# REXJJ/high-fidelity-pointcloud-fusion

Measured on AMD Instinct MI355X. Metric: Mpts/s fused into 1 mm voxel grid, higher is better.
Workload: dtype f64

## Files before the change

### high-fidelity-pointcloud-fusion_amd/csrc/hfpf.hip

```cpp
#include <hip/hip_runtime.h>

#include <cstring>

#include <rocprim/rocprim.hpp>

#include <dlfcn.h>
#include <sched.h>
#include <sys/mman.h>

#if !defined(__HIP_DEVICE_COMPILE__)
#include <emmintrin.h>
#endif
#include <algorithm>
#include <atomic>
#include <condition_variable>
#include <cmath>
#include <cstdarg>
#include <cstdio>
#include <cstdlib>
#include <cstring>
#include <mutex>
#include <string>
#include <thread>
#include <vector>
// ... 115 lines not shown
                }
            }
            if (stop_.load(std::memory_order_acquire)) return;
            seen = g;
            part(i);
            remaining_.fetch_sub(1, std::memory_order_acq_rel);
        }
    }
    std::vector<std::thread> th_;
    std::mutex m_;
    std::condition_variable cv_;
    std::atomic<uint64_t> gen_{0};
    std::atomic<int> remaining_{0}, sleepers_{0};
    std::atomic<bool> stop_{false};
    char* dst_ = nullptr;
    const char* src_ = nullptr;
    size_t bytes_ = 0;
};

constexpr int kStageSlots = 8;
constexpr size_t kXferChunk = 16u << 20;
#ifndef HFPF_PROBE_FRAMES
#define HFPF_PROBE_FRAMES 8
#endif
constexpr int kProbeFrames = HFPF_PROBE_FRAMES;
constexpr int kFrameSlots = 8;

struct DepthSpec {
    uint32_t width, height, depth_f32, depth_step, color_bpp, color_bgr, color_step;
    float cx, cy, sx, sy, unit;
    uint32_t color_off;
    size_t depth_bytes() const { return (size_t)(height - 1) * depth_step + (size_t)width * (depth_f32 ? 4u : 2u); }
    size_t color_bytes() const { return color_bpp ? (size_t)(height - 1) * color_step + (size_t)width * color_bpp : 0; }
};
static_assert(sizeof(DepthSpec) == 13 * 4, "DepthSpec is compared bytewise");

DepthLayout depth_layout(const DepthSpec& d, const void* dev_color, uint64_t color_stride)
{
    return DepthLayout{d.color_bpp ? (const uint8_t*)dev_color : nullptr, color_stride, d.width, d.depth_step, d.color_step, d.depth_f32,
                       d.color_bpp, d.color_bgr, d.cx, d.cy, d.sx, d.sy, d.unit};
}

struct Knobs {
    int copy_streams = 2;
    bool update_cells = true;
    int host_batch = 4;
    int upd_shape_forced = -1;
    bool trace_shape = false;
    bool bin_spare = true;
    bool stream_replay = true;
    float bin_slack = 2.0f;
    bool clean_small_nowait = true;
    bool clean_overlap = true;
    bool trace_clean = false;
    float test_bin_scale = 1.f;
    bool test_table_skip = false;
    bool mailbox = true;
    int test_dev_tile = kDevTileDefault;
    int stage_threads = 0;
};

struct Session {
    bool dirty = false;
    uint64_t n_linked[kLogRegions] = {0};
    uint64_t gate_done = 0;
    bool pend_valid = false;
    uint64_t direct_linked = 0;
    bool normals_possible = false;
    uint32_t next_frame_id = 0;
    bool poisoned = false;
    std::string poison_msg;
    bool bin_have_hist = false;
    bool bin_from_probe = false;
    double bin_prev_points = 0;
    uint64_t n_bricks_known = 0;
    uint64_t n_bricks_before = 0;
    unsigned long long upd_miss_seen = 0, upd_member_seen = 0;
    unsigned long long pub_seq = 0;
    unsigned long long early_seq = 0;
    unsigned long long win_seq = 0;
    uint32_t pend_n = 0, pend_first = 0;
    uint32_t pend_pts = 0;
    uint32_t pend_lay[5] = {0, 0, 0, 0, 0};
    bool pend_depth = false;
    DepthSpec pend_ds{};
    double pend_pose[kFrameSlots * 12] = {0};
    uint64_t occ_exported = 0;
    uint64_t frames_exported = 0, frames_seen = 0;
};

constexpr int kTimeIntegrate = 0, kTimeClean = 1, kTimeDetail = 2, kTimeRaycast = 5, kTimeComponents = 6, kTimeCompare = 7, kTimedIds = 8;
struct TimedId {
    std::vector<std::pair<hipEvent_t, hipEvent_t>> pending;
    double ms = 0;
    uint64_t n = 0;
};

}

struct hfpf_handle {
    std::mutex mtx;
    std::string err;

    hfpf_config cfg;
    GridParams g;
    Knobs knobs;
    bool binned = false;
    int integrate_grid = 1536;
    size_t dir_entries = 0;
    uint64_t n_slots = 0;
    uint64_t max_touched = 0;

    Session ss;
    uint64_t frames_integrated = 0;
    uint64_t clean_passes = 0;
    uint32_t launch_seq = 0;
    bool upd_wide = false;
    bool epoch_used = false;
    unsigned long long mbox_seq = 0;
    int stage_next = 0, fslot_next = 0;

    Tables t;
    hipStream_t stream = nullptr;
    hipStream_t copy_stream = nullptr;
    hipStream_t copy_more[3] = {nullptr, nullptr, nullptr};
    std::vector<void*> allocs;
    uint64_t device_bytes = 0;
    unsigned long long* h_ctr = nullptr;
    unsigned long long* h_log_ctr = nullptr;
    unsigned long long* mbox = nullptr;
    hipStream_t front_stream = nullptr;
    hipEvent_t ev_ready = nullptr, ev_front = nullptr;
    std::vector<DevBuf*> bufs;
    DevBuf pend_a{bufs}, pend_b{bufs};
    StageSlot stage[kStageSlots];
    FrameSlot fslot[kFrameSlots];
    void* ring_d = nullptr;
    size_t ring_cap = 0;
    hipEvent_t busy_ev = nullptr;
    bool busy_pending = false;
    void* xfer_pin[2] = {nullptr, nullptr};
    hipEvent_t xfer_ev[2] = {nullptr, nullptr};
    StagePool* stage_pool = nullptr;
    DevBuf sort_tmp{bufs}, keys_a{bufs}, keys_b{bufs}, vals_a{bufs}, vals_b{bufs}, rows_dev{bufs};
    DevBuf probe_a{bufs}, probe_b{bufs}, probe_c{bufs}, probe_d{bufs}, probe_e{bufs}, probe_f{bufs};
    DevBuf result_out{bufs};
    DevBuf zbuf{bufs}, render_pose{bufs}, render_out{bufs};
    DevBuf track_in{bufs};
    DevBuf icp_acc{bufs};
    DevBuf query_in{bufs}, query_out{bufs};
    DevBuf mesh_cube{bufs}, mesh_corner{bufs}, mesh_kdata{bufs}, mesh_cdata{bufs}, mesh_ctr{bufs};
    DevBuf comp_index{bufs}, comp_rows{bufs}, comp_recs{bufs};
    DevBuf dev_mesh{bufs}, dev_tri{bufs}, dev_bins{bufs}, dev_pairs{bufs};
    DevBuf align_dev{bufs};
    DevBuf cov_bins{bufs};
    DevBuf ray_in{bufs}, ray_out{bufs}, ray_map{bufs};
    DevBuf snap_stage{bufs}, snap_err{bufs};
    uint64_t bin_pool = 0;
    DevBuf bin_pt_buf{bufs}, bin_rgb_buf{bufs}, bin_sums{bufs};
    DevBuf ovf_pt_buf{bufs}, ovf_aux_buf{bufs};
    bool dist_on = false;
    int rank = 0, world = 1;
    void* rccl_lib = nullptr;
    void* comm = nullptr;
    uint64_t ex_cap_records = 0;
    DevBuf ex_send{bufs}, ex_recv{bufs}, ex_counts{bufs}, stats_total{bufs};
    unsigned long long* h_counts = nullptr;

    bool timing = false;
    bool timing_detail = false;
    std::vector<hipEvent_t> ev_detail;
    std::vector<uint8_t> ev_detail_ran;
    TimedId timed[kTimedIds];
    std::vector<hipEvent_t> ev_free;
};

namespace {

int fail(hfpf_handle* h, int code, const char* fmt, ...)
{
    char buf[512];
    va_list ap;
    va_start(ap, fmt);
    vsnprintf(buf, sizeof buf, fmt, ap);
    va_end(ap);
// ... 153 lines not shown
    unsigned long long upd_tested = 0, upd_member = 0;
    for (int r = 0; r < kLogRegions; r++) {
        upd_tested += h->h_log_ctr[r * 16 + 2];
        upd_member += h->h_log_ctr[r * 16 + 3];
    }
    h->h_ctr[C_DEP_TESTED] += upd_tested;
    h->h_ctr[C_DEP_MEMBER] += upd_member;
    unsigned long long single = 0;
    for (int r = 0; r < kLogRegions; r++) single += h->h_log_ctr[r * 16 + 4];
    h->h_ctr[C_TOUCHED_SINGLE] = single;
    {
        const uint64_t nbk = std::min<uint64_t>(h->h_ctr[C_BRICKS], h->t.max_bricks);
        if (nbk != h->ss.n_bricks_known) h->ss.n_bricks_before = h->ss.n_bricks_known;
        h->ss.n_bricks_known = nbk;
    }
    return HFPF_OK;
}

int check_device_errors(hfpf_handle* h)
{
    const unsigned long long e = h->h_ctr[C_ERR];
    if (!e) return HFPF_OK;
    std::string what;
    if (e & E_BRICKS) what += " brick pool (max_bricks)";
    if (e & E_LOG) what += " point log (max_log_points)";
    if (e & E_OCC) what += " occupied list (max_normals*4)";
    if (e & E_NORMALS) what += " normal records (max_normals)";
    if (e & E_REG) what += " registrations (max_normals*7)";
    if (e & E_DEP) what += " dependant table";
    if (e & E_SPIN) what += " brick-claim spin bound";
    if (e & E_DEPCNT) what += " more than 65535 dependants on one cell";
    if (e & E_FRAME) what += " frame id >= max_frames";
    if (e & E_OVF) what += " integrate overflow list";
    if (e & E_CHAIN) what += " point-log chain / run record out of range (internal)";
    return fail(h, HFPF_ERR_CAPACITY, "device pool overflow:%s", what.c_str());
}

float stat_scale_for(double bound) { return (float)std::ldexp(1.0, 26 - (int)std::floor(std::log2(bound))); }

Knobs read_knobs()
{
    Knobs k;
    if (const char* cs = getenv("HFPF_COPY_STREAMS")) k.copy_streams = std::max(1, std::min(atoi(cs), 4));
    const char* uf = getenv("HFPF_UPDATE_FORM");
    k.update_cells = !(uf && uf[0] == 'p');
    if (const char* hb = getenv("HFPF_HOST_BATCH")) k.host_batch = std::max(1, std::min(atoi(hb), kFrameSlots));
    if (const char* us = getenv("HFPF_UPD_SHAPE")) k.upd_shape_forced = std::max(0, std::min(atoi(us), 1));
    if (const char* tr = getenv("HFPF_TRACE_SHAPE")) k.trace_shape = tr[0] != '0';
    if (const char* sp = getenv("HFPF_BIN_SPARE")) k.bin_spare = sp[0] != '0';
    if (const char* sr = getenv("HFPF_STREAM_REPLAY")) k.stream_replay = sr[0] != '0';
    if (const char* bs = getenv("HFPF_BIN_SLACK")) k.bin_slack = std::max(1.0f, std::min(4.0f, (float)atof(bs)));
    if (const char* nw = getenv("HFPF_CLEAN_NOWAIT")) k.clean_small_nowait = nw[0] != '0';
    if (const char* co = getenv("HFPF_CLEAN_OVERLAP")) k.clean_overlap = co[0] != '0';
    if (const char* tc = getenv("HFPF_TRACE_CLEAN")) k.trace_clean = tc[0] != '0';
    if (const char* bs = getenv("HFPF_TEST_BIN_SCALE")) k.test_bin_scale = std::max(0.f, std::min(1.f, (float)atof(bs)));
    const char* ts = getenv("HFPF_TEST_TABLE_SKIP");
    k.test_table_skip = ts && ts[0] == '1';
    if (const char* dt = getenv("HFPF_TEST_DEV_TILE")) k.test_dev_tile = std::max(8, std::min(atoi(dt), kDevTileMax));
    const char* mb = getenv("HFPF_MAILBOX");
    k.mailbox = !mb || mb[0] != '0';
    int cores = (int)std::thread::hardware_concurrency();
    cpu_set_t set;
    if (sched_getaffinity(0, sizeof set, &set) == 0) cores = std::min(cores > 0 ? cores : 1 << 20, CPU_COUNT(&set));
    const char* st = getenv("HFPF_STAGE_THREADS");
    k.stage_threads = st ? std::max(0, std::min(atoi(st), 15)) : std::max(0, std::min(7, cores / 2 - 1));
    return k;
}

int setup_params(hfpf_handle* h)
{
    const hfpf_config& c = h->cfg;
    GridParams& g = h->g;
    if (!(c.resolution > 0.f)) return fail(h, HFPF_ERR_BAD_CONFIG, "resolution must be > 0");
    for (int a = 0; a < 3; a++)
        if (!(c.bbox[2 * a + 1] > c.bbox[2 * a])) return fail(h, HFPF_ERR_BAD_CONFIG, "bounding_box axis %d: max <= min", a);
    if (c.k != 2) return fail(h, HFPF_ERR_BAD_CONFIG, "k must be 2 (the reference probes exactly 125 neighbours, OccupancyGrid.hpp:334)");
    if (c.K < 0 || c.K > 16) return fail(h, HFPF_ERR_BAD_CONFIG, "K out of range [0,16]");
    if (!(c.cylinder_radius > 0) || !(c.ball_radius > 0)) return fail(h, HFPF_ERR_BAD_CONFIG, "radii must be > 0");
    g.res = (double)c.resolution;
    g.inv_res = 1.0 / g.res;
    for (int a = 0; a < 3; a++) {
        g.min[a] = c.bbox[2 * a];
        g.max[a] = c.bbox[2 * a + 1];
        const double d = (g.max[a] - g.min[a]) / g.res;
        if (!(d < 2097151.0)) return fail(h, HFPF_ERR_BAD_CONFIG, "axis %d: more than 2^21 cells", a);
        g.dim[a] = (int32_t)d;
        g.bdim[a] = (g.dim[a] + 1 + 7) / 8;
    }
    {
        auto bits_for = [](int32_t dim) {
            uint32_t b = 1;
            while ((1ll << b) <= (long long)dim) b++;
            return b;
        };
        g.key_sy = bits_for(g.dim[2]);
        g.key_sx = g.key_sy + bits_for(g.dim[1]);
        g.key_bits = g.key_sx + bits_for(g.dim[0]);
    }
    g.zclip_min = c.z_clip_min;
    g.zclip_max = c.z_clip_max;
    {
        auto float_at_or_above = [](double m) {
            float f = (float)m;
            if ((double)f < m) f = nextafterf(f, INFINITY);
            return f;
        };
// ... 787 lines not shown
    if (n >= (1ull << 20))
        hipLaunchKernelGGL(k_gate<4>, dim3(blocks_for(n, 256 * 4)), dim3(256), 0, s, h->g, h->t, cells_a, n_a, cells_b, n_b, pend_out);
    else
        hipLaunchKernelGGL(k_gate<1>, dim3(blocks_for(n, 256)), dim3(256), 0, s, h->g, h->t, cells_a, n_a, cells_b, n_b, pend_out);
}

int clean_locked(hfpf_handle* h, int pre_rc)
{
    Tables& t = h->t;
    hipStream_t s = h->stream;
    int rc;
    if (h->dist_on && (rc = dist_exchange_locked(h, pre_rc))) return rc;
    if (pre_rc) return pre_rc;
    const bool early = h->knobs.clean_overlap && !h->dist_on && h->binned && h->mbox && h->ss.pub_seq && h->ss.early_seq;
    if ((rc = read_counters(h, early))) return rc;
    if ((rc = check_device_errors(h))) return rc;
    const uint64_t n_occ = std::min<uint64_t>(h->h_ctr[C_OCC], t.max_occ);
    const uint64_t n_normals = h->h_ctr[C_NORMALS];
    const uint64_t n_pend = h->ss.pend_valid ? h->h_ctr[C_PEND] : 0;
    h->ss.occ_exported = n_occ;
    h->ss.frames_exported = std::max(h->ss.frames_exported, h->ss.frames_seen);
    h->ss.dirty = false;
    h->clean_passes++;

    {
        LinkRanges lr;
        uint64_t max_new = 0;
        for (int r = 0; r < kLogRegions; r++) {
            const uint64_t n_r = std::min<uint64_t>(h->h_log_ctr[r * 16], t.log_region_cap);
            const uint64_t base = (uint64_t)r * t.log_region_cap;
            lr.first[r] = (uint32_t)(base + h->ss.n_linked[r] + 1);
            lr.last[r] = (uint32_t)(base + n_r);
            max_new = std::max(max_new, n_r - h->ss.n_linked[r]);
            h->ss.n_linked[r] = n_r;
        }
        if (max_new && !h->binned && h->h_ctr[C_BUFFERED] != h->ss.direct_linked) {
            hipLaunchKernelGGL(k_link_log, dim3(blocks_for(max_new, 256), kLogRegions), dim3(256), 0, s, t, lr);
            HIPCHK(h, hipGetLastError());
        }
        h->ss.direct_linked = h->h_ctr[C_BUFFERED];
    }
    if (n_occ == 0) return HFPF_OK;

    const uint64_t n_new_occ = n_occ - std::min(n_occ, h->ss.gate_done);
    const uint64_t n_in = n_pend + n_new_occ;
    if (n_in == 0) return HFPF_OK;
    if ((rc = scratch(h, h->pend_b, n_in * 4))) return rc;
    if ((rc = scratch(h, h->keys_a, n_in * 8))) return rc;
    const uint64_t reg_ub = (2ull * (uint64_t)h->g.K + 1ull) * n_in;
    const uint64_t live_ub = std::min<uint64_t>(h->h_ctr[C_REG], t.max_reg) + std::min<uint64_t>(h->h_ctr[C_PREREG], t.max_reg);
    bool full = h->h_ctr[C_DEP] + 2 * live_ub + 2 * reg_ub + n_new_occ > t.max_dep;
    const bool overlap = early && !full;
    const uint32_t* new_cells = (const uint32_t*)(t.occ_list + h->ss.gate_done);
    if (h->knobs.trace_clean)
        fprintf(stderr, "hfpf: clean pass %llu: %llu candidates, front half %s\n", (unsigned long long)h->clean_passes, (unsigned long long)n_in,
                overlap ? "beside the update kernel" : "on the engine's stream");
    if (overlap) {
        s = h->front_stream;
        HIPCHK(h, hipStreamWaitEvent(s, h->ev_ready, 0));
        hipLaunchKernelGGL(k_clean_front, dim3(blocks_for(n_in, 256)), dim3(256), 0, s, t, n_in);
    } else {
        hipLaunchKernelGGL(k_clean_begin, dim3(blocks_for(n_in, 256)), dim3(256), 0, s, t, n_in, new_cells, n_new_occ, full ? 1u : 0u);
    }
    launch_gate(h, s, (const uint32_t*)h->pend_a.p, n_pend, new_cells, n_new_occ, (uint32_t*)h->pend_b.p);
    HIPCHK(h, hipGetLastError());
    h->ss.gate_done = n_occ;
    h->ss.normals_possible = true;
    swap(h->pend_a, h->pend_b);
    h->ss.pend_valid = true;

    const unsigned cand_bits = HFPF_MORTON_IDS ? 3u * std::max(h->g.key_sy, std::max(h->g.key_sx - h->g.key_sy, h->g.key_bits - h->g.key_sx)) : h->g.key_bits;
    if ((rc = sort_keys_u64(h, t.cand_key, (uint64_t*)h->keys_a.p, n_in, cand_bits, s))) return rc;
    hipLaunchKernelGGL(k_normal, dim3(blocks_for(n_in, 128)), dim3(128), 0, s, h->g, t, (const uint64_t*)h->keys_a.p, kCountOnDevice, n_normals);
    const bool reg_small = n_in < (1ull << 18);
    const uint64_t reg_tile = 256ull * (reg_small ? kRegTilesSmall : kRegTilesLarge);
    const uint64_t reg_blocks = ((n_in + reg_tile - 1) / reg_tile) * (2ull * (uint64_t)h->g.K + 1ull);
    const uint32_t count_deps = full ? 0u : 1u;
    if (reg_small) hipLaunchKernelGGL(k_register<kRegTilesSmall>, dim3((unsigned)std::max<uint64_t>(reg_blocks, 1)), dim3(256), 0, s, h->g, t, kCountOnDevice, n_normals, count_deps);
    else hipLaunchKernelGGL(k_register<kRegTilesLarge>, dim3((unsigned)std::max<uint64_t>(reg_blocks, 1)), dim3(256), 0, s, h->g, t, kCountOnDevice, n_normals, count_deps);
    HIPCHK(h, hipGetLastError());
    if (overlap) {
        HIPCHK(h, hipEventRecord(h->ev_front, s));
        s = h->stream;
        HIPCHK(h, hipStreamWaitEvent(s, h->ev_front, 0));
        if (n_new_occ) hipLaunchKernelGGL(k_clean_file, dim3(blocks_for(n_new_occ, 256)), dim3(256), 0, s, t, new_cells, n_new_occ);
    }
    uint64_t n_reg = 0, n_pre = 0, inc_touched = 0;
    const uint64_t reg_first = std::min<uint64_t>(h->h_ctr[C_REG], t.max_reg);
    const bool no_wait = !full && reg_ub < (1ull << 21) && h->knobs.clean_small_nowait;
    if (!full) {
        hipLaunchKernelGGL(k_depinc_offsets, dim3(blocks_for(reg_ub, 256 * kListTiles)), dim3(256), 0, s, t, kCountOnDevice);
        hipLaunchKernelGGL(k_depinc_fill, dim3(blocks_for(reg_ub, 256)), dim3(256), 0, s, t, reg_first, kCountOnDevice);
        HIPCHK(h, hipGetLastError());
        if (no_wait) {
            with_color(t.color, [&](auto C) {
                hipLaunchKernelGGL(k_replay<C>, dim3(blocks_for(reg_ub * kChains, 256)), dim3(256), 0, s, h->g, t, (const uint32_t*)t.touched_list, 1u, 0u,
                                   kCountOnDevice, n_normals);
            });
            HIPCHK(h, hipGetLastError());
            return HFPF_OK;
        }
        if ((rc = read_counters(h))) return rc;
        n_reg = std::min<uint64_t>(h->h_ctr[C_REG], t.max_reg);
        n_pre = std::min<uint64_t>(h->h_ctr[C_PREREG], t.max_reg);
        inc_touched = h->h_ctr[C_TOUCHED];
        if (h->h_ctr[C_ERR] == (unsigned long long)E_DEP) {
            hipLaunchKernelGGL(k_set_ctr, dim3(1), dim3(1), 0, s, t.ctr, (int)C_ERR, 0ull);
            if (inc_touched) hipLaunchKernelGGL(k_dep_reset, dim3(blocks_for(inc_touched, 256)), dim3(256), 0, s, t, inc_touched);
            full = true;
        } else if ((rc = check_device_errors(h))) {
            return rc;
        }
    } else {
        if ((rc = read_counters(h))) return rc;
        if ((rc = check_device_errors(h))) return rc;
        n_reg = std::min<uint64_t>(h->h_ctr[C_REG], t.max_reg);
        n_pre = std::min<uint64_t>(h->h_ctr[C_PREREG], t.max_reg);
    }
    if (full) {
        const uint64_t n_all = n_reg + n_pre;
        if (2 * n_all > t.max_dep)
            return fail(h, HFPF_ERR_CAPACITY, "dependant table: %llu entries do not fit %llu with their blocks", (unsigned long long)n_all, (unsigned long long)t.max_dep);
        if (n_all > h->max_touched) return fail(h, HFPF_ERR_CAPACITY, "registrations: %llu > %llu", (unsigned long long)n_all, (unsigned long long)h->max_touched);
        hipLaunchKernelGGL(k_set_ctr3, dim3(1), dim3(1), 0, s, t.ctr, (int)C_DEP, 0ull, (int)C_TOUCHED, 0ull, -1, 0ull);
        if (n_all) {
            hipLaunchKernelGGL(k_dep_count, dim3(blocks_for(n_all, 256)), dim3(256), 0, s, t, n_reg, n_pre);
            HIPCHK(h, hipGetLastError());
            if ((rc = read_counters(h))) return rc;
            const uint64_t n_touched = h->h_ctr[C_TOUCHED];
            hipLaunchKernelGGL(k_dep_offsets, dim3(blocks_for(n_touched, 256)), dim3(256), 0, s, t, n_touched);
            hipLaunchKernelGGL(k_dep_fill, dim3(blocks_for(n_all, 256)), dim3(256), 0, s, t, n_reg, n_pre);
            hipLaunchKernelGGL(k_dep_reset, dim3(blocks_for(n_touched, 256)), dim3(256), 0, s, t, n_touched);
            HIPCHK(h, hipGetLastError());
            inc_touched = n_touched;
        }
        if ((rc = read_counters(h))) return rc;
        if ((rc = check_device_errors(h))) return rc;
    }
    if (inc_touched) {
        const uint32_t use_marks = full ? 0u : 1u;
        const uint64_t single = full ? 0 : std::min<uint64_t>(h->h_ctr[C_TOUCHED_SINGLE], inc_touched);
        const bool stream = !full && h->binned && h->knobs.stream_replay && single >= (1ull << 16);
        if (stream) {
            const uint32_t nbk = (uint32_t)h->ss.n_bricks_known;
            const bool wide = h->knobs.upd_shape_forced >= 0 ? h->knobs.upd_shape_forced == 1 : h->upd_wide;
            launch_update_cells<true>(t.color, wide, s, h->g, t, nbk);
// ... 15 lines not shown
            HIPCHK(h, hipGetLastError());
        }
    }
    return HFPF_OK;
}

}

extern "C" {

int hfpf_abi_version(void) { return HFPF_ABI_VERSION; }

void hfpf_default_config(hfpf_config* c)
{
    if (!c) return;
    memset(c, 0, sizeof *c);
    c->struct_size = sizeof *c;
    c->resolution = 0.005f;
    const double box[6] = {-0.80, 1.80, -1.5, 1.5, 0.0, 1.0};
    memcpy(c->bbox, box, sizeof box);
    c->k = 2;
    c->K = 3;
    c->gate = 20;
    c->cylinder_radius = 0.001;
    c->ball_radius = 0.015;
    c->z_clip_min = 0.28;
    c->z_clip_max = 0.6;
    c->device = 0;
}

const char* hfpf_last_error(const hfpf_handle* h) { return h ? h->err.c_str() : g_create_error.c_str(); }

int hfpf_create(const hfpf_config* cfg, hfpf_handle** out)
{
    if (!cfg || !out) return fail(nullptr, HFPF_ERR_BAD_ARG, "hfpf_create: null argument");
    if (cfg->struct_size != sizeof(hfpf_config)) return fail(nullptr, HFPF_ERR_BAD_CONFIG, "hfpf_config.struct_size mismatch (ABI %d)", HFPF_ABI_VERSION);
    *out = nullptr;
    hfpf_handle* h = new hfpf_handle();
    h->cfg = *cfg;
    h->knobs = read_knobs();
    auto bail = [&](int rc) {
        g_create_error = h->err;
        for (void* p : h->allocs) (void)hipFree(p);
        for (DevBuf* b : h->bufs)
            if (b->p) (void)hipFree(b->p);
        if (h->h_ctr) (void)hipHostFree(h->h_ctr);
        if (h->h_log_ctr) (void)hipHostFree(h->h_log_ctr);
        if (h->mbox) (void)hipHostFree(h->mbox);
        if (h->copy_stream) (void)hipStreamDestroy(h->copy_stream);
        for (hipStream_t cs : h->copy_more)
            if (cs) (void)hipStreamDestroy(cs);
        if (h->ev_ready) (void)hipEventDestroy(h->ev_ready);
        if (h->ev_front) (void)hipEventDestroy(h->ev_front);
        if (h->front_stream) (void)hipStreamDestroy(h->front_stream);
        if (h->stream) (void)hipStreamDestroy(h->stream);
        delete h;
        return rc;
    };
    int rc = setup_params(h);
    if (rc) return bail(rc);
    int ndev = 0;
    hipError_t e = hipGetDeviceCount(&ndev);
    if (e != hipSuccess || ndev <= 0) return bail(fail(h, HFPF_ERR_HIP, "no HIP device available (%s); this engine has no CPU path", hipGetErrorString(e)));
    if (cfg->device < 0 || cfg->device >= ndev) return bail(fail(h, HFPF_ERR_BAD_CONFIG, "device %d out of range (%d devices)", cfg->device, ndev));
    if ((e = hipSetDevice(cfg->device)) != hipSuccess) return bail(fail(h, HFPF_ERR_HIP, "hipSetDevice: %s", hipGetErrorString(e)));
    if ((e = hipStreamCreateWithFlags(&h->stream, hipStreamNonBlocking)) != hipSuccess) return bail(fail(h, HFPF_ERR_HIP, "hipStreamCreate: %s", hipGetErrorString(e)));
    if ((e = hipStreamCreateWithFlags(&h->copy_stream, hipStreamNonBlocking)) != hipSuccess) return bail(fail(h, HFPF_ERR_HIP, "hipStreamCreate: %s", hipGetErrorString(e)));
    for (int k = 0; k + 1 < h->knobs.copy_streams; k++)
        if ((e = hipStreamCreateWithFlags(&h->copy_more[k], hipStreamNonBlocking)) != hipSuccess) return bail(fail(h, HFPF_ERR_HIP, "hipStreamCreate: %s", hipGetErrorString(e)));
    if ((e = hipStreamCreateWithFlags(&h->front_stream, hipStreamNonBlocking)) != hipSuccess) return bail(fail(h, HFPF_ERR_HIP, "hipStreamCreate: %s", hipGetErrorString(e)));
    if ((e = hipEventCreateWithFlags(&h->ev_ready, hipEventDisableTiming)) != hipSuccess || (e = hipEventCreateWithFlags(&h->ev_front, hipEventDisableTiming)) != hipSuccess)
        return bail(fail(h, HFPF_ERR_HIP, "hipEventCreate: %s", hipGetErrorString(e)));
    if ((e = hipHostMalloc((void**)&h->h_ctr, C_COUNT * sizeof(unsigned long long), hipHostMallocDefault)) != hipSuccess)
        return bail(fail(h, HFPF_ERR_HIP, "hipHostMalloc: %s", hipGetErrorString(e)));
    memset(h->h_ctr, 0, C_COUNT * sizeof(unsigned long long));
    if ((e = hipHostMalloc((void**)&h->h_log_ctr, kLogRegions * 16 * sizeof(unsigned long long), hipHostMallocDefault)) != hipSuccess)
        return bail(fail(h, HFPF_ERR_HIP, "hipHostMalloc: %s", hipGetErrorString(e)));
    memset(h->h_log_ctr, 0, kLogRegions * 16 * sizeof(unsigned long long));
    if (h->knobs.mailbox) {
        if ((e = hipHostMalloc((void**)&h->mbox, 2 * kMboxSlotWords * sizeof(unsigned long long), hipHostMallocCoherent | hipHostMallocMapped)) != hipSuccess)
            return bail(fail(h, HFPF_ERR_HIP, "hipHostMalloc (mailbox): %s", hipGetErrorString(e)));
        memset(h->mbox, 0, 2 * kMboxSlotWords * sizeof(unsigned long long));
    }
    {
        int per_cu = 0, cus = 0;
        hipDeviceProp_t prop;
        if (hipGetDeviceProperties(&prop, cfg->device) == hipSuccess) cus = prop.multiProcessorCount;
        if (hipOccupancyMaxActiveBlocksPerMultiprocessor(&per_cu, h->binned ? k_integrate<true, false, true> : k_integrate<true, false, false>, 256, 0) != hipSuccess) per_cu = 4;
        h->integrate_grid = std::max(1, per_cu) * std::max(1, cus);
    }
    if ((rc = alloc_tables(h))) return bail(rc);
    {
        const uint64_t n0 = h->cfg.max_normals;
        if ((rc = scratch(h, h->keys_a, n0 * 8)) || (rc = scratch(h, h->keys_b, n0 * 8)) || (rc = scratch(h, h->vals_a, n0 * 4)) ||
            (rc = scratch(h, h->vals_b, n0 * 4)) || (rc = scratch(h, h->pend_b, n0 * 4)) || (rc = scratch(h, h->sort_tmp, n0 * 16)))
            return bail(rc);
        if (h->cfg.max_call_points && h->binned) {
            const uint64_t pts = h->cfg.max_call_points;
            const uint64_t pool = std::min<uint64_t>(bin_pool_entries(h, pts, h->cfg.max_bricks), 0xFFFFFFFFull);
            if ((rc = scratch(h, h->bin_pt_buf, pool * sizeof(float4)))) return bail(rc);
            if (h->t.color && (rc = scratch(h, h->bin_rgb_buf, pool * 4))) return bail(rc);
            h->bin_pool = pool;
            if ((rc = scratch(h, h->ovf_pt_buf, pts * sizeof(float4))) || (rc = scratch(h, h->ovf_aux_buf, pts * sizeof(uint2)))) return bail(rc);
        }
    }
    for (int k = 0; k < 2; k++) {
        if (hipHostMalloc(&h->xfer_pin[k], kXferChunk, hipHostMallocDefault) != hipSuccess || hipEventCreateWithFlags(&h->xfer_ev[k], hipEventDisableTiming) != hipSuccess) {
            (void)hipGetLastError();
            if (h->xfer_pin[0]) (void)hipHostFree(h->xfer_pin[0]);
            h->xfer_pin[0] = nullptr;
            break;
        }
    }
    if ((e = hipStreamSynchronize(h->stream)) != hipSuccess) return bail(fail(h, HFPF_ERR_HIP, "sync after init: %s", hipGetErrorString(e)));
    *out = h;
    return HFPF_OK;
}

int hfpf_destroy(hfpf_handle* h)
{
    if (!h) return HFPF_OK;
    (void)hipSetDevice(h->cfg.device);
    (void)hipStreamSynchronize(h->stream);
    if (h->front_stream) (void)hipStreamSynchronize(h->front_stream);
    for (void* p : h->allocs) (void)hipFree(p);
    for (DevBuf* b : h->bufs)
        if (b->p) (void)hipFree(b->p);
    if (h->comm && g_rccl.CommDestroy) (void)g_rccl.CommDestroy((ncclComm_t_)h->comm);
    if (h->h_counts) (void)hipHostFree(h->h_counts);
    for (auto& s : h->stage) {
        if (s.h_pose) (void)hipHostFree(s.h_pose);
        if (s.d_pose) (void)hipFree(s.d_pose);
        if (s.done) (void)hipEventDestroy(s.done);
    }
    delete h->stage_pool;
    h->stage_pool = nullptr;
    for (int k = 0; k < 2; k++) {
        if (h->xfer_pin[k]) (void)hipHostFree(h->xfer_pin[k]);
        if (h->xfer_ev[k]) (void)hipEventDestroy(h->xfer_ev[k]);
    }
    for (auto& f : h->fslot) {
        if (f.h) (void)hipHostFree(f.h);
        if (f.done) (void)hipEventDestroy(f.done);
        if (f.copied) (void)hipEventDestroy(f.copied);
    }
    if (h->ring_d) (void)hipFree(h->ring_d);
    if (h->busy_ev) (void)hipEventDestroy(h->busy_ev);
    if (h->copy_stream) {
        (void)hipStreamSynchronize(h->copy_stream);
        (void)hipStreamDestroy(h->copy_stream);
    }
    for (hipStream_t cs : h->copy_more)
        if (cs) {
            (void)hipStreamSynchronize(cs);
            (void)hipStreamDestroy(cs);
        }
    for (TimedId& t : h->timed)
        for (auto& pr : t.pending) {
            (void)hipEventDestroy(pr.first);
            (void)hipEventDestroy(pr.second);
        }
    for (auto e : h->ev_detail) (void)hipEventDestroy(e);
    for (auto e : h->ev_free) (void)hipEventDestroy(e);
    if (h->h_ctr) (void)hipHostFree(h->h_ctr);
    if (h->h_log_ctr) (void)hipHostFree(h->h_log_ctr);
    if (h->mbox) (void)hipHostFree(h->mbox);
    if (h->ev_ready) (void)hipEventDestroy(h->ev_ready);
    if (h->ev_front) (void)hipEventDestroy(h->ev_front);
    if (h->front_stream) (void)hipStreamDestroy(h->front_stream);
    if (h->stream) (void)hipStreamDestroy(h->stream);
    delete h;
    return HFPF_OK;
}

int hfpf_get_dims(const hfpf_handle* h, int32_t dims[3], double* resolution)
{
    if (!h) return HFPF_ERR_BAD_ARG;
    if (dims) memcpy(dims, h->g.dim, 3 * sizeof(int32_t));
    if (resolution) *resolution = h->g.res;
    return HFPF_OK;
}

static int flush_pending_locked(hfpf_handle* h);

int hfpf_integrate_device(hfpf_handle* h, const void* dev_base, uint32_t n_frames, uint64_t frame_stride, uint32_t n_points, uint32_t point_step,
                          uint32_t off_x, uint32_t off_y, uint32_t off_z, uint32_t off_rgb, const double* poses, const uint32_t* frame_ids)
{
    if (!h) return HFPF_ERR_BAD_ARG;
    std::lock_guard<std::mutex> lk(h->mtx);
    HIPCHK(h, hipSetDevice(h->cfg.device));
    if (int rcf = flush_pending_locked(h)) return rcf;
    if (int rc = check_usable(h)) return rc;
    return integrate_device_locked(h, dev_base, n_frames, frame_stride, n_points, point_step, off_x, off_y, off_z, off_rgb, poses, frame_ids);
}

static void host_copy(hfpf_handle* h, void* dst, const void* src, size_t bytes)
{
    if (h->knobs.stage_threads > 0 && bytes >= (1u << 20)) {
        if (!h->stage_pool) h->stage_pool = new StagePool(h->knobs.stage_threads);
        h->stage_pool->copy(dst, src, bytes);
    } else {
        stream_copy((char*)dst, (const char*)src, bytes);
    }
}

static int flush_pending_locked(hfpf_handle* h)
{
    if (h->ss.pend_n == 0) return HFPF_OK;
    const uint32_t first = h->ss.pend_first, n = h->ss.pend_n;
    h->ss.pend_n = 0;
    if (h->ss.poisoned) return fail(h, HFPF_ERR_STATE, "%u accepted host frame(s) dropped: handle failed earlier (%s); hfpf_clear resets it", n, h->ss.poison_msg.c_str());
    for (uint32_t k = n, seen = 0; k-- > 0;) {
        const uint32_t which = (first + k) % (uint32_t)h->knobs.copy_streams;
        if (seen & (1u << which)) continue;
        seen |= 1u << which;
        HIPCHK(h, hipStreamWaitEvent(h->stream, h->fslot[first + k].copied, 0));
    }
    const char* ring = (const char*)h->ring_d + (size_t)first * h->ring_cap;
    const DepthLayout dl = depth_layout(h->ss.pend_ds, ring + h->ss.pend_ds.color_off, h->ring_cap);
    int rc = integrate_device_locked(h, ring, n, h->ring_cap, h->ss.pend_pts, h->ss.pend_lay[0], h->ss.pend_lay[1], h->ss.pend_lay[2], h->ss.pend_lay[3],
                                     h->ss.pend_lay[4], h->ss.pend_pose, nullptr, h->ss.pend_depth ? &dl : nullptr);
// ... 3101 lines not shown
```

### high-fidelity-pointcloud-fusion_amd/csrc/kernels.hpp

```cpp
#pragma once
#include <type_traits>

#include "stats.hpp"

namespace hfpf {

typedef float vf4 __attribute__((ext_vector_type(4)));

struct FrameLayout {
    uint32_t point_step, off_x, off_y, off_z, off_rgb;
};

struct DepthLayout {
    const uint8_t* color;
    uint64_t color_stride;
    uint32_t width, depth_step, color_step;
    uint32_t depth_f32;
    uint32_t color_bpp;
    uint32_t color_bgr;
    float cx, cy, sx, sy, unit;
};

template <bool WANT_RGB>
__device__ __forceinline__ vf4 depth_fetch(const uint8_t* __restrict__ dimg, const uint8_t* __restrict__ cimg, const DepthLayout& L, uint32_t i)
// ... 1528 lines not shown
        for (int k = 0; k < B; k++) {
            stat_delta_zero(d[k]);
            ldv[k] = line_div_of(ldd[k]);
        }
        if (any) {
            uint32_t e = head;
            while (e) {
                const float4 p = t.log_pt[e];
                const uint32_t rgb = COLOR ? t.log_rgb[e] : 0u;
                const F3 pt = F3{p.x, p.y, p.z};
#pragma unroll
                for (int k = 0; k < B; k++) {
                    if (use[k]) {
                        float sp, distf;
                        if (line_member_hoisted(g, pt, la[k], lab[k], ldv[k], sp, distf)) stat_delta_add(d[k], pair_delta(g, sp, distf), rgb);
                    }
                }
                e = __float_as_uint(p.w);
            }
        }
#pragma unroll
        for (int k = 0; k < B; k++) {
#pragma unroll
            for (int w = 0; w < kStatUsed; w++) {
                long long v = d[k].v[w];
#pragma unroll
                for (uint32_t o = 1; o < kChains; o <<= 1) v += __shfl_xor(v, (int)o);
                d[k].v[w] = v;
            }
            if constexpr (COLOR) {
#pragma unroll
                for (int w = 0; w < 3; w++) {
                    long long v = d[k].rgb[w];
#pragma unroll
                    for (uint32_t o = 1; o < kChains; o <<= 1) v += __shfl_xor(v, (int)o);
                    d[k].rgb[w] = v;
                }
            }
            const bool member = sub == 0 && d[k].v[SW_COUNT] != 0;
            if (member) replayed += (uint32_t)d[k].v[SW_COUNT];
            wave_flush_members(t, q, member, d[k], sid[k]);
        }
    }
    __shared__ unsigned int s_rep;
    if (threadIdx.x == 0) s_rep = 0;
    __syncthreads();
#pragma unroll
    for (int o = 32; o > 0; o >>= 1) replayed += __shfl_down(replayed, o);
    if ((threadIdx.x & 63u) == 0 && replayed) atomicAdd(&s_rep, replayed);
    __syncthreads();
    if (threadIdx.x == 0 && s_rep) atomicAdd(&t.log_ctr[(blockIdx.x & (kLogRegions - 1)) * 16 + 1], (unsigned long long)s_rep);
}

__device__ __forceinline__ uint32_t reg_slot(const Tables& t, uint64_t j, uint64_t n_reg) { return j < n_reg ? t.reg_occ[j].x : t.prereg_list[j - n_reg]; }

__device__ __forceinline__ uint32_t dep_capacity(uint32_t cnt) { return cnt <= 1u ? cnt : 1u << (32 - __clz((int)(cnt - 1u))); }

__global__ __launch_bounds__(256) void k_dep_count(const Tables t, const uint64_t n_reg, const uint64_t n_pre)
{
    const uint64_t j = (uint64_t)blockIdx.x * blockDim.x + threadIdx.x;
    bool fresh = false;
    uint32_t slot = 0;
    if (j < n_reg + n_pre) {
        slot = reg_slot(t, j, n_reg);
        fresh = atomicAdd(&t.dep_tmp[slot], 1u) == 0u;
    }
    __shared__ BlockReserveScratch brs;
    const unsigned long long ti = block_reserve(&t.ctr[C_TOUCHED], fresh, brs);
    if (fresh) t.touched_list[ti] = slot;
}

__global__ __launch_bounds__(256) void k_dep_offsets(const Tables t, const uint64_t n_touched)
{
    const uint64_t j = (uint64_t)blockIdx.x * blockDim.x + threadIdx.x;
    const bool act = j < n_touched;
    const uint32_t slot = act ? t.touched_list[j] : 0u;
    uint32_t cnt = act ? t.dep_tmp[slot] : 0u;
    if (cnt > kDepCntMask) {
        atomicOr(&t.ctr[C_ERR], (unsigned long long)E_DEPCNT);
        cnt = (uint32_t)kDepCntMask;
    }
    const unsigned long long off = wave_reserve_n(&t.ctr[C_DEP], dep_capacity(cnt));
    if (!act) return;
    t.info[slot] = (t.info[slot] & 3ull) | ((uint64_t)cnt << kDepCntShift) | ((uint64_t)off << kDepOffShift);
    if (cnt) set_dep_flag(t, slot);
    t.dep_tmp[slot] = 0;
}

__global__ __launch_bounds__(256) void k_dep_fill(const Tables t, const uint64_t n_reg, const uint64_t n_pre)
{
    const uint64_t j = (uint64_t)blockIdx.x * blockDim.x + threadIdx.x;
    if (j >= n_reg + n_pre) return;
    const uint32_t slot = reg_slot(t, j, n_reg);
    const uint32_t nid = j < n_reg ? t.reg_occ[j].y : t.pre_dep[slot];
    const uint64_t info = t.info[slot];
    const uint32_t k = atomicAdd(&t.dep_tmp[slot], 1u);
    if (k >= ((info >> kDepCntShift) & kDepCntMask)) return;
    t.dep[(info >> kDepOffShift) + k] = make_dep_entry(t, nid);
}

__global__ __launch_bounds__(256) void k_dep_reset(const Tables t, const uint64_t n_touched)
{
    const uint64_t n = n_touched == kCountOnDevice ? (uint64_t)t.ctr[C_TOUCHED] : n_touched;
    const uint64_t j = (uint64_t)blockIdx.x * blockDim.x + threadIdx.x;
    if (j < n) t.dep_tmp[t.touched_list[j]] = 0;
}
// ... 2 lines not shown

__global__ __launch_bounds__(256) void k_depinc_offsets(const Tables t, const uint64_t n_touched_arg)
{
    const uint64_t n_touched = n_touched_arg == kCountOnDevice ? (uint64_t)t.ctr[C_TOUCHED] : n_touched_arg;
    uint32_t slot_[kListTiles], old_cnt_[kListTiles], new_cnt_[kListTiles], take_[kListTiles];
    uint64_t info_[kListTiles];
#pragma unroll
    for (int tt = 0; tt < kListTiles; tt++) {
        const uint64_t j = ((uint64_t)blockIdx.x * kListTiles + tt) * 256u + threadIdx.x;
        slot_[tt] = 0, old_cnt_[tt] = 0, new_cnt_[tt] = 0, take_[tt] = 0, info_[tt] = 0;
        if (j < n_touched) {
            slot_[tt] = t.touched_list[j];
            info_[tt] = t.info[slot_[tt]];
            old_cnt_[tt] = (uint32_t)((info_[tt] >> kDepCntShift) & kDepCntMask);
            new_cnt_[tt] = old_cnt_[tt] + t.dep_tmp[slot_[tt]];
            if (new_cnt_[tt] > dep_capacity(old_cnt_[tt])) take_[tt] = dep_capacity(min(new_cnt_[tt], (uint32_t)kDepCntMask));
        }
    }
    __shared__ TileReserveScratch<kListTiles> trs;
    unsigned long long off_[kListTiles];
    uint32_t n_single = 0;
    block_reserve_tiles<kListTiles>(&t.ctr[C_DEP], take_, off_, trs);
#pragma unroll
    for (int tt = 0; tt < kListTiles; tt++) {
        const uint64_t j = ((uint64_t)blockIdx.x * kListTiles + tt) * 256u + threadIdx.x;
        if (j >= n_touched) continue;
        const uint32_t slot = slot_[tt], old_cnt = old_cnt_[tt], new_cnt = new_cnt_[tt];
        const uint64_t info = info_[tt], old_off = info >> kDepOffShift;
        const bool moves = take_[tt] != 0;
        const unsigned long long off = moves ? off_[tt] : old_off;
        if ((moves && off + take_[tt] > t.max_dep) || new_cnt > kDepCntMask || old_cnt > kDepOldMax) {
            atomicOr(&t.ctr[C_ERR], (unsigned long long)(new_cnt > kDepCntMask ? E_DEPCNT : E_DEP));
            t.dep_tmp[slot] = kDepPoison;
            continue;
        }
        n_single += t.run_cnt[slot >> 9] == 1u ? 1u : 0u;
        if (moves) {
            for (uint32_t k = 0; k < old_cnt; k++) t.dep[off + k] = t.dep[old_off + k];
        }
        t.info[slot] = (info & 3ull) | ((uint64_t)new_cnt << kDepCntShift) | ((uint64_t)off << kDepOffShift);
        if (old_cnt == 0 && new_cnt) set_dep_flag(t, slot);
        t.dep_tmp[slot] = (old_cnt << 16) | old_cnt;
    }
    __shared__ unsigned int s_single;
    if (threadIdx.x == 0) s_single = 0;
    __syncthreads();
#pragma unroll
    for (int o = 32; o > 0; o >>= 1) n_single += __shfl_down(n_single, o);
    if ((threadIdx.x & 63u) == 0 && n_single) atomicAdd(&s_single, n_single);
    __syncthreads();
    if (threadIdx.x == 0 && s_single) atomicAdd(&t.log_ctr[(blockIdx.x & (kLogRegions - 1)) * 16 + 4], (unsigned long long)s_single);
}

__global__ __launch_bounds__(256) void k_depinc_fill(const Tables t, const uint64_t reg_first, const uint64_t n_reg_arg)
{
    const uint64_t n_reg = n_reg_arg == kCountOnDevice ? min((uint64_t)t.ctr[C_REG], t.max_reg) : n_reg_arg;
    const uint64_t j = reg_first + (uint64_t)blockIdx.x * blockDim.x + threadIdx.x;
    if (j >= n_reg) return;
    const uint2 r = t.reg_occ[j];
    const uint32_t v = atomicAdd(&t.dep_tmp[r.x], 1u);
    if (v & kDepPoison) return;
    const uint32_t k = v & 0xFFFFu;
    const uint64_t info = t.info[r.x];
    t.dep[(info >> kDepOffShift) + k] = make_dep_entry(t, r.y);
    if (k + 1 == (uint32_t)((info >> kDepCntShift) & kDepCntMask)) t.dep_tmp[r.x] = kTouchedMark | ((v >> 16) & kDepOldMax);
}


struct ExtractOpts {
    double min_count;
    int32_t classify_threshold;
    int32_t paint_white;
};
constexpr int kExtractTiles = 8;
__global__ __launch_bounds__(256) void k_extract_keys(const GridParams g, const Tables t, const unsigned long long* __restrict__ stats,
                                                      const uint64_t n_normals, const ExtractOpts opt, uint64_t* __restrict__ keys,
                                                      uint32_t* __restrict__ vals)
{
    __shared__ unsigned int s_rows;
    if (threadIdx.x == 0) s_rows = 0;
    __syncthreads();
    uint32_t n_valid = 0;
#pragma unroll
    for (int tt = 0; tt < kExtractTiles; tt++) {
        const uint64_t j = ((uint64_t)blockIdx.x * kExtractTiles + tt) * 256u + threadIdx.x;
        if (j >= n_normals) continue;
        const uint64_t nid = j + 1;
        const uint64_t key = t.nv_key[nid];
        int32_t x, y, z;
        key_coords(g, key, x, y, z);
        uint32_t valid = valid_coord(g, x, y, z) ? 1u : 0u;
        if (valid && opt.min_count > 0.0) {
            const long long cnt = (long long)stats[nid * kStatWords + SW_COUNT];
            if ((double)(int)cnt < opt.min_count) valid = 0;
        }
        keys[j] = valid ? key : ~0ull;
        vals[j] = (uint32_t)nid;
        n_valid += valid;
    }
#pragma unroll
    for (int o = 32; o > 0; o >>= 1) n_valid += __shfl_down(n_valid, o);
    if ((threadIdx.x & 63u) == 0 && n_valid) atomicAdd(&s_rows, n_valid);
    __syncthreads();
    if (threadIdx.x == 0 && s_rows) atomicAdd(&t.ctr[C_ROWS], (unsigned long long)s_rows);
}

struct Row {
    int32_t ix, iy, iz;
    uint32_t count;
    float x, y, z;
    float nx, ny, nz;
    float sdx, sdy, sdz;
    float mean_dist, sd_dist;
    uint32_t rgb;
};
static_assert(sizeof(Row) == 64, "row is 64 bytes");

__device__ __forceinline__ void record_centroid(const GridParams& g, const Tables& t, const long long* s, const uint64_t nid, const long long cnt,
// ... 2143 lines not shown
```

Baseline: 29060.

## Replay new registrations on the front stream beside the dependant-table update

Adds a k_replay_reg kernel that replays buffered log points directly from the registration list on the front stream, so it runs concurrently with the depinc offsets/fill kernels instead of waiting behind them. When enabled, k_depinc_fill clears dep_tmp rather than leaving a touched note, and the main stream waits on a new event and returns early, skipping the touched-list replay. This shortens the serial chain in small clean passes but adds a stream dependency and changes how touched-slot state is left for later passes.

```diff
diff --git a/high-fidelity-pointcloud-fusion_amd/csrc/hfpf.hip b/high-fidelity-pointcloud-fusion_amd/csrc/hfpf.hip
--- a/high-fidelity-pointcloud-fusion_amd/csrc/hfpf.hip
+++ b/high-fidelity-pointcloud-fusion_amd/csrc/hfpf.hip
@@ -191,6 +191,7 @@
     float bin_slack = 2.0f;
     bool clean_small_nowait = true;
     bool clean_overlap = true;
+    bool early_replay = true;
     bool trace_clean = false;
     float test_bin_scale = 1.f;
     bool test_table_skip = false;
@@ -269,7 +270,7 @@
     unsigned long long* h_log_ctr = nullptr;
     unsigned long long* mbox = nullptr;
     hipStream_t front_stream = nullptr;
-    hipEvent_t ev_ready = nullptr, ev_front = nullptr;
+    hipEvent_t ev_ready = nullptr, ev_front = nullptr, ev_replay = nullptr;
     std::vector<DevBuf*> bufs;
     DevBuf pend_a{bufs}, pend_b{bufs};
     StageSlot stage[kStageSlots];
@@ -529,6 +530,7 @@
     if (const char* bs = getenv("HFPF_BIN_SLACK")) k.bin_slack = std::max(1.0f, std::min(4.0f, (float)atof(bs)));
     if (const char* nw = getenv("HFPF_CLEAN_NOWAIT")) k.clean_small_nowait = nw[0] != '0';
     if (const char* co = getenv("HFPF_CLEAN_OVERLAP")) k.clean_overlap = co[0] != '0';
+    if (const char* er = getenv("HFPF_EARLY_REPLAY")) k.early_replay = er[0] != '0';
     if (const char* tc = getenv("HFPF_TRACE_CLEAN")) k.trace_clean = tc[0] != '0';
     if (const char* bs = getenv("HFPF_TEST_BIN_SCALE")) k.test_bin_scale = std::max(0.f, std::min(1.f, (float)atof(bs)));
     const char* ts = getenv("HFPF_TEST_TABLE_SKIP");
@@ -1422,9 +1424,12 @@
     bool full = h->h_ctr[C_DEP] + 2 * live_ub + 2 * reg_ub + n_new_occ > t.max_dep;
     const bool overlap = early && !full;
     const uint32_t* new_cells = (const uint32_t*)(t.occ_list + h->ss.gate_done);
+    const uint64_t reg_first = std::min<uint64_t>(h->h_ctr[C_REG], t.max_reg);
+    const bool no_wait = !full && reg_ub < (1ull << 21) && h->knobs.clean_small_nowait;
+    const bool replay_early = overlap && no_wait && h->knobs.early_replay;
     if (h->knobs.trace_clean)
-        fprintf(stderr, "hfpf: clean pass %llu: %llu candidates, front half %s\n", (unsigned long long)h->clean_passes, (unsigned long long)n_in,
-                overlap ? "beside the update kernel" : "on the engine's stream");
+        fprintf(stderr, "hfpf: clean pass %llu: %llu candidates, front half %s, replay %s\n", (unsigned long long)h->clean_passes, (unsigned long long)n_in,
+                overlap ? "beside the update kernel" : "on the engine's stream", replay_early ? "fed from the registrations" : "behind the dependant-table update");
     if (overlap) {
         s = h->front_stream;
         HIPCHK(h, hipStreamWaitEvent(s, h->ev_ready, 0));
@@ -1451,17 +1456,26 @@
     HIPCHK(h, hipGetLastError());
     if (overlap) {
         HIPCHK(h, hipEventRecord(h->ev_front, s));
+        if (replay_early) {
+            with_color(t.color, [&](auto C) {
+                hipLaunchKernelGGL(k_replay_reg<C>, dim3(blocks_for(reg_ub * kChains, 256)), dim3(256), 0, s, h->g, t, reg_first, kCountOnDevice);
+            });
+            HIPCHK(h, hipGetLastError());
+            HIPCHK(h, hipEventRecord(h->ev_replay, s));
+        }
         s = h->stream;
         HIPCHK(h, hipStreamWaitEvent(s, h->ev_front, 0));
         if (n_new_occ) hipLaunchKernelGGL(k_clean_file, dim3(blocks_for(n_new_occ, 256)), dim3(256), 0, s, t, new_cells, n_new_occ);
     }
     uint64_t n_reg = 0, n_pre = 0, inc_touched = 0;
-    const uint64_t reg_first = std::min<uint64_t>(h->h_ctr[C_REG], t.max_reg);
-    const bool no_wait = !full && reg_ub < (1ull << 21) && h->knobs.clean_small_nowait;
     if (!full) {
         hipLaunchKernelGGL(k_depinc_offsets, dim3(blocks_for(reg_ub, 256 * kListTiles)), dim3(256), 0, s, t, kCountOnDevice);
-        hipLaunchKernelGGL(k_depinc_fill, dim3(blocks_for(reg_ub, 256)), dim3(256), 0, s, t, reg_first, kCountOnDevice);
+        hipLaunchKernelGGL(k_depinc_fill, dim3(blocks_for(reg_ub, 256)), dim3(256), 0, s, t, reg_first, kCountOnDevice, replay_early ? 0u : 1u);
         HIPCHK(h, hipGetLastError());
+        if (replay_early) {
+            HIPCHK(h, hipStreamWaitEvent(s, h->ev_replay, 0));
+            return HFPF_OK;
+        }
         if (no_wait) {
             with_color(t.color, [&](auto C) {
                 hipLaunchKernelGGL(k_replay<C>, dim3(blocks_for(reg_ub * kChains, 256)), dim3(256), 0, s, h->g, t, (const uint32_t*)t.touched_list, 1u, 0u,
@@ -1583,6 +1597,7 @@
             if (cs) (void)hipStreamDestroy(cs);
         if (h->ev_ready) (void)hipEventDestroy(h->ev_ready);
         if (h->ev_front) (void)hipEventDestroy(h->ev_front);
+        if (h->ev_replay) (void)hipEventDestroy(h->ev_replay);
         if (h->front_stream) (void)hipStreamDestroy(h->front_stream);
         if (h->stream) (void)hipStreamDestroy(h->stream);
         delete h;
@@ -1600,7 +1615,8 @@
     for (int k = 0; k + 1 < h->knobs.copy_streams; k++)
         if ((e = hipStreamCreateWithFlags(&h->copy_more[k], hipStreamNonBlocking)) != hipSuccess) return bail(fail(h, HFPF_ERR_HIP, "hipStreamCreate: %s", hipGetErrorString(e)));
     if ((e = hipStreamCreateWithFlags(&h->front_stream, hipStreamNonBlocking)) != hipSuccess) return bail(fail(h, HFPF_ERR_HIP, "hipStreamCreate: %s", hipGetErrorString(e)));
-    if ((e = hipEventCreateWithFlags(&h->ev_ready, hipEventDisableTiming)) != hipSuccess || (e = hipEventCreateWithFlags(&h->ev_front, hipEventDisableTiming)) != hipSuccess)
+    if ((e = hipEventCreateWithFlags(&h->ev_ready, hipEventDisableTiming)) != hipSuccess || (e = hipEventCreateWithFlags(&h->ev_front, hipEventDisableTiming)) != hipSuccess ||
+        (e = hipEventCreateWithFlags(&h->ev_replay, hipEventDisableTiming)) != hipSuccess)
         return bail(fail(h, HFPF_ERR_HIP, "hipEventCreate: %s", hipGetErrorString(e)));
     if ((e = hipHostMalloc((void**)&h->h_ctr, C_COUNT * sizeof(unsigned long long), hipHostMallocDefault)) != hipSuccess)
         return bail(fail(h, HFPF_ERR_HIP, "hipHostMalloc: %s", hipGetErrorString(e)));
@@ -1698,6 +1714,7 @@
     if (h->mbox) (void)hipHostFree(h->mbox);
     if (h->ev_ready) (void)hipEventDestroy(h->ev_ready);
     if (h->ev_front) (void)hipEventDestroy(h->ev_front);
+    if (h->ev_replay) (void)hipEventDestroy(h->ev_replay);
     if (h->front_stream) (void)hipStreamDestroy(h->front_stream);
     if (h->stream) (void)hipStreamDestroy(h->stream);
     delete h;
diff --git a/high-fidelity-pointcloud-fusion_amd/csrc/kernels.hpp b/high-fidelity-pointcloud-fusion_amd/csrc/kernels.hpp
--- a/high-fidelity-pointcloud-fusion_amd/csrc/kernels.hpp
+++ b/high-fidelity-pointcloud-fusion_amd/csrc/kernels.hpp
@@ -1604,6 +1604,70 @@
     if (threadIdx.x == 0 && s_rep) atomicAdd(&t.log_ctr[(blockIdx.x & (kLogRegions - 1)) * 16 + 1], (unsigned long long)s_rep);
 }
 
+template <bool COLOR>
+__global__ __launch_bounds__(256) void k_replay_reg(const GridParams g, const Tables t, const uint64_t reg_first, const uint64_t n_reg_arg)
+{
+    __shared__ unsigned long long queue[4][kQueueRows * kQueueStride];
+    __shared__ unsigned int s_rep;
+    const uint64_t n_reg = n_reg_arg == kCountOnDevice ? min((uint64_t)t.ctr[C_REG], t.max_reg) : n_reg_arg;
+    if (reg_first + (uint64_t)blockIdx.x * (256u / kChains) >= n_reg) return;
+    unsigned long long* q = queue[threadIdx.x >> 6];
+    const uint64_t gid = (uint64_t)blockIdx.x * blockDim.x + threadIdx.x;
+    const uint64_t j = reg_first + gid / kChains;
+    const uint32_t sub = (uint32_t)(gid % kChains);
+    uint32_t nid = 0, head = 0;
+    if (j < n_reg) {
+        const uint2 r = t.reg_occ[j];
+        nid = r.y;
+        head = t.buf_head[(uint64_t)r.x * kChains + sub];
+    }
+    uint32_t any = head;
+#pragma unroll
+    for (uint32_t o = 1; o < kChains; o <<= 1) any |= (uint32_t)__shfl_xor((int)any, (int)o);
+    StatDeltaT<COLOR> d;
+    stat_delta_zero(d);
+    if (any) {
+        float4 e0, e1;
+        pre_list_entry(t, nid, e0, e1);
+        const F3 la = F3{e0.y, e0.z, e0.w}, lab = F3{e1.x, e1.y, e1.z};
+        const LineDiv ldv = line_div_of(e1.w);
+        uint32_t e = head;
+        while (e) {
+            const float4 p = t.log_pt[e];
+            const uint32_t rgb = COLOR ? t.log_rgb[e] : 0u;
+            float sp, distf;
+            if (line_member_hoisted(g, F3{p.x, p.y, p.z}, la, lab, ldv, sp, distf)) stat_delta_add(d, pair_delta(g, sp, distf), rgb);
+            e = __float_as_uint(p.w);
+        }
+    }
+#pragma unroll
+    for (int w = 0; w < kStatUsed; w++) {
+        long long v = d.v[w];
+#pragma unroll
+        for (uint32_t o = 1; o < kChains; o <<= 1) v += __shfl_xor(v, (int)o);
+        d.v[w] = v;
+    }
+    if constexpr (COLOR) {
+#pragma unroll
+        for (int w = 0; w < 3; w++) {
+            long long v = d.rgb[w];
+#pragma unroll
+            for (uint32_t o = 1; o < kChains; o <<= 1) v += __shfl_xor(v, (int)o);
+            d.rgb[w] = v;
+        }
+    }
+    const bool member = sub == 0 && d.v[SW_COUNT] != 0;
+    uint32_t replayed = member ? (uint32_t)d.v[SW_COUNT] : 0u;
+    wave_flush_members(t, q, member, d, nid);
+    if (threadIdx.x == 0) s_rep = 0;
+    __syncthreads();
+#pragma unroll
+    for (int o = 32; o > 0; o >>= 1) replayed += __shfl_down(replayed, o);
+    if ((threadIdx.x & 63u) == 0 && replayed) atomicAdd(&s_rep, replayed);
+    __syncthreads();
+    if (threadIdx.x == 0 && s_rep) atomicAdd(&t.log_ctr[(blockIdx.x & (kLogRegions - 1)) * 16 + 1], (unsigned long long)s_rep);
+}
+
 __device__ __forceinline__ uint32_t reg_slot(const Tables& t, uint64_t j, uint64_t n_reg) { return j < n_reg ? t.reg_occ[j].x : t.prereg_list[j - n_reg]; }
 
 __device__ __forceinline__ uint32_t dep_capacity(uint32_t cnt) { return cnt <= 1u ? cnt : 1u << (32 - __clz((int)(cnt - 1u))); }
@@ -1712,7 +1776,7 @@
     if (threadIdx.x == 0 && s_single) atomicAdd(&t.log_ctr[(blockIdx.x & (kLogRegions - 1)) * 16 + 4], (unsigned long long)s_single);
 }
 
-__global__ __launch_bounds__(256) void k_depinc_fill(const Tables t, const uint64_t reg_first, const uint64_t n_reg_arg)
+__global__ __launch_bounds__(256) void k_depinc_fill(const Tables t, const uint64_t reg_first, const uint64_t n_reg_arg, const uint32_t leave_note)
 {
     const uint64_t n_reg = n_reg_arg == kCountOnDevice ? min((uint64_t)t.ctr[C_REG], t.max_reg) : n_reg_arg;
     const uint64_t j = reg_first + (uint64_t)blockIdx.x * blockDim.x + threadIdx.x;
@@ -1723,7 +1787,7 @@
     const uint32_t k = v & 0xFFFFu;
     const uint64_t info = t.info[r.x];
     t.dep[(info >> kDepOffShift) + k] = make_dep_entry(t, r.y);
-    if (k + 1 == (uint32_t)((info >> kDepCntShift) & kDepCntMask)) t.dep_tmp[r.x] = kTouchedMark | ((v >> 16) & kDepOldMax);
+    if (k + 1 == (uint32_t)((info >> kDepCntShift) & kDepCntMask)) t.dep_tmp[r.x] = leave_note ? kTouchedMark | ((v >> 16) & kDepOldMax) : 0u;
 }
 
 
```

Measured after the change: 30470, median of 6. +4.8%, better.
